# sangminwoo/Temporal-Span-Proposal-Network-VidVRD

Measured on AMD Instinct MI355X. Metric: tracklet-pairs/sec scored (N=32, T=150, D=2048), higher is better.
Workload: dtype f32

## Files before the change

include/tspn_mi355x.h:

```cpp
#ifndef TSPN_MI355X_H
#define TSPN_MI355X_H

#include <stddef.h>
#include <stdint.h>

#ifdef __cplusplus
extern "C" {
#endif

#define TSPN_ABI_VERSION 7

enum {
  TSPN_OK = 0,
  TSPN_EINVAL = -1,
  TSPN_EUNSUPPORTED = -2,
  TSPN_EWORKSPACE = -3,
  TSPN_ELAUNCH = -4,
  TSPN_EDEVICE = -5
};

#define TSPN_STATUS_WORDS 16
enum {
  TSPN_STATUS_FAULT = 0,
  TSPN_STATUS_FAULT_INFO = 1,
// ... 84 lines not shown
size_t tspn_conv3_tc_wino63_workspace_bytes(int64_t B, int64_t T, int64_t Cin);
int tspn_conv3_tc_wino63_f32(const float* x, int64_t B, int64_t T, int64_t Cin, const float* frag,
                             int64_t M, const float* bias, int relu, float* y,
                             void* workspace, size_t workspace_bytes, void* stream);
int tspn_conv3_tc_wino63_set_piece_form(int form);

size_t tspn_pack_conv3_wino63_f16x3_elements(int64_t M, int64_t Cin, int64_t split);
int tspn_pack_conv3_wino63_f16x3(const float* W, int64_t M, int64_t Cin, int64_t split, int16_t* packed, void* stream);
size_t tspn_conv3_tc_wino63_f16x3_workspace_bytes(int64_t B, int64_t T, int64_t Cin, int64_t M);
int tspn_conv3_tc_wino63_f16x3(const float* x, int64_t B, int64_t T, int64_t Cin, const int16_t* packed,
                               int64_t M, const float* bias, int relu, float* y,
                               void* workspace, size_t workspace_bytes, void* stream);
int tspn_conv3_tc_wino63_f16x3_set_tail_split(int on);


int tspn_heads_f32(int mode, const float* a, const float* b, int64_t lda,
                   const int64_t* ia, const int64_t* ib, int64_t idx_stride, const float* bias,
                   const float* Wh, const float* bh, int64_t H,
                   int64_t P, int64_t C, int64_t T, float* out, void* stream);

int tspn_heads_pairgrid_f32(const float* y, int64_t B, int64_t N, int64_t C, int64_t T,
                            const float* Wh, const float* bh, int64_t H, float* out,
                            void* stream);

int tspn_temporal_mean_f32(const float* x, int64_t R, int64_t T, int64_t Cdim,
                           int layout_tc, float* out, void* stream);
int tspn_temporal_sum_f32(const float* x, int64_t R, int64_t T, int64_t Cdim, float* out, void* stream);

int tspn_pair_rows_f32(const float* src, int64_t NT, int64_t D, const int64_t* pairs,
                       int64_t P, float* out, void* stream);

int tspn_transpose_td_f32(const float* x, int64_t R, int64_t T, int64_t D, float* out,
                          void* stream);

size_t tspn_decode_topk_workspace_bytes(int64_t S, int64_t P, int64_t topk_pair);
int tspn_decode_topk_f32(const float* rel_logit, const int64_t* pairs,
                         const float* cls_sub, const float* cls_obj, int64_t ld,
                         int64_t seg_rows, int64_t row_mul, int64_t S, int64_t P, int64_t K,
                         int64_t NO, int64_t topk_pair, int64_t topk_seg,
                         float* out_score, int64_t* out_triplet, int64_t* out_pair_tid,
                         void* workspace, size_t workspace_bytes, void* stream);

int tspn_decode_spans_f32(const float* heads, int64_t P, int64_t A, int64_t T,
                          const float* sizes_host, int64_t top_k, double nms_threshold,
                          int64_t pre_nms, int64_t* out_anchor, int64_t* out_span,
                          float* out_span_f, float* out_score, int64_t* out_count, void* stream);
// ... 216 lines not shown
```

temporal-span-proposal-network-vidvrd_amd/_abi.py:

```python
import ctypes
import os
import re
import threading

HERE = os.path.dirname(os.path.abspath(__file__))
ROOT = os.path.dirname(HERE)
LIB_PATH = os.environ.get("TSPN_LIB_PATH") or os.path.join(HERE, "libtspn_mi355x.so")
HEADER_PATH = os.path.join(ROOT, "include", "tspn_mi355x.h")

ABI_VERSION = 7
TSPN_OK = 0
TSPN_EINVAL = -1
TSPN_EUNSUPPORTED = -2
TSPN_EWORKSPACE = -3
TSPN_ELAUNCH = -4
TSPN_EDEVICE = -5
STATUS_WORDS = 16
STATUS_FAULT, STATUS_FAULT_INFO, STATUS_CONV_ERR, STATUS_CONV_CHECKS = 0, 1, 2, 3
FAULT_HANDOVER = 1
CONV_CHECK_HOT_OFFSET, CONV_CHECK_SCRATCH_BYTES = 256, 256 + 256 * 64
GEOM_CHANNELS = 8
CONV_DIRECT, CONV_WINOGRAD63, CONV_WINOGRAD63_F16X3 = 0, 1, 2

_c_f32p = ctypes.c_void_p
# ... 45 lines not shown
    "tspn_status_selftest": (_int, [_vp, _vp]),
    "tspn_conv3_spot_check_f32": (_int, [_vp, _i64, _i64, _i64, _vp, _i64, _i64, _i64, _vp, _int, _vp, _i64, _vp, _i64, _vp]),
    "tspn_predicate_head_workspace_bytes": (_sz, [_i64, _i64, _i64]),
    "tspn_predicate_head_f32": (_int, [_vp, _i64, _i64, _i64, _vp, _vp, _i64, _vp, _int, _vp, _sz, _vp]),
    "tspn_predicate_head_norm_workspace_bytes": (_sz, [_i64, _i64, _i64, _i64, _i64, _i64]),
    "tspn_predicate_head_norm_f32": (_int, [_vp, _i64, _i64, _i64, _vp, _vp, _i64, _i64, _i64, _i64, _vp, _int,
                                            _vp, _sz, _vp]),
    "tspn_feature_preprocess_f32": (_int, [_vp, _i64, _i64, _i64, _i64, _i64, _i64, _vp]),
    "tspn_proposal_pair_filter_i64": (_int, [_vp, _vp, _vp, _vp, _i64, _vp, _vp, _vp, _vp]),
    "tspn_gather_rows_f32": (_int, [_vp, _i64, _i64, _vp, _i64, _i64, _vp, _vp]),
    "tspn_ppn_pair_matrix_topk_f32": (_int, [_vp, _i64, _i64, _i64, _i64, _i64,
                                             _vp, _vp, _vp, _vp, _vp, _vp, _vp, _vp,
                                             _i64, _vp, _vp, _vp]),
    "tspn_traj_iou_f32": (_int, [_vp, _i64, _vp, _i64, _i64, _i64, _vp, _vp]),
    "tspn_traj_iou_tail_f64": (_int, [_vp, _vp, _vp, _i64, _i64, _i64, _vp, _vp]),
    "tspn_pair_index_i64": (_int, [_i64, _i64, _vp, _vp]),
    "tspn_pair_gather_f32": (_int, [_vp, _vp, _i64, _i64, _i64, _vp, _i64, _vp, _vp, _vp]),
    "tspn_pack_conv3_f32": (_int, [_vp, _i64, _i64, _i64, _vp, _vp]),
    "tspn_conv3_f32": (_int, [_vp, _i64, _i64, _i64, _vp, _i64, _vp, _int, _vp, _vp]),
    "tspn_conv3_tc_f32": (_int, [_vp, _i64, _i64, _i64, _vp, _i64, _vp, _int, _vp, _vp]),
    "tspn_heads_f32": (_int, [_int, _vp, _vp, _i64, _vp, _vp, _i64, _vp, _vp, _vp, _i64, _i64, _i64,
                              _i64, _vp, _vp]),
    "tspn_heads_pairgrid_f32": (_int, [_vp, _i64, _i64, _i64, _i64, _vp, _vp, _i64, _vp, _vp]),
    "tspn_temporal_mean_f32": (_int, [_vp, _i64, _i64, _i64, _int, _vp, _vp]),
    "tspn_temporal_sum_f32": (_int, [_vp, _i64, _i64, _i64, _vp, _vp]),
    "tspn_pair_rows_f32": (_int, [_vp, _i64, _i64, _vp, _i64, _vp, _vp]),
    "tspn_transpose_td_f32": (_int, [_vp, _i64, _i64, _i64, _vp, _vp]),
    "tspn_decode_topk_workspace_bytes": (_sz, [_i64, _i64, _i64]),
    "tspn_decode_topk_f32": (_int, [_vp, _vp, _vp, _vp, _i64, _i64, _i64, _i64, _i64, _i64, _i64, _i64, _i64,
                                    _vp, _vp, _vp, _vp, _sz, _vp]),
    "tspn_decode_spans_f32": (_int, [_vp, _i64, _i64, _i64, ctypes.POINTER(ctypes.c_float), _i64,
                                     ctypes.c_double, _i64, _vp, _vp, _vp, _vp, _vp, _vp]),
    "tspn_forward_fused_workspace_bytes": (_sz, [ctypes.POINTER(FusedDesc)]),
    "tspn_forward_fused_f32": (_int, [ctypes.POINTER(FusedDesc), _vp]),
    "tspn_temporal_encoder_heads_f32": (_int, [_vp, _i64, _i64, _i64, _vp, _vp, _vp, _vp, _i64,
                                               _vp, _vp, _vp]),
    "tspn_pack_conv2d_f32": (_int, [_vp, _i64, _i64, _i64, _i64, _vp, _vp]),
    "tspn_conv2d_nhwc_f32": (_int, [_vp, _i64, _i64, _i64, _i64, _vp, _i64, _i64, _i64, _i64, _i64, _vp, _vp,
                                    _int, _vp, _vp]),
    "tspn_pack_conv2d_frag_f32": (_int, [_vp, _i64, _i64, _i64, _i64, _vp, _vp]),
    "tspn_conv2d_nhwc_frag_f32": (_int, [_vp, _i64, _i64, _i64, _i64, _vp, _i64, _i64, _i64, _i64, _i64, _vp, _vp,
                                         _int, _vp, _vp]),
    "tspn_pack_conv2d_frag_bf16": (_int, [_vp, _i64, _i64, _i64, _i64, _vp, _vp]),
    "tspn_conv2d_nhwc_bf16": (_int, [_vp, _i64, _i64, _i64, _i64, _vp, _i64, _i64, _i64, _i64, _i64, _vp, _vp,
                                     _int, _vp, _vp]),
    "tspn_roi_align_nhwc_f32": (_int, [_vp, _i64, _i64, _i64, _i64, _vp, _i64, _i64, ctypes.c_float, _int, _int,
# ... 123 lines not shown
```

temporal-span-proposal-network-vidvrd_amd/build.py:

```python
import glob
import json
import os
import re
import shutil
import subprocess
import sys

HERE = os.path.dirname(os.path.abspath(__file__))
ROOT = os.path.dirname(HERE)
CSRC = os.path.join(HERE, "csrc")
CSRC_EVAL = os.path.join(CSRC, "eval")
CSRC_REL = os.path.join(CSRC, "relations")
CSRC_PAIRLIST = os.path.join(CSRC, "pairlist")
CSRC_SPANBF16 = os.path.join(CSRC, "spanbf16")
CSRC_SPANLOSS = os.path.join(CSRC, "spanloss")
LIB_NAME = "libtspn_mi355x.so"
LIB_PATH = os.path.join(HERE, LIB_NAME)
ARCH = "gfx950"

FLAGS = [
    f"--offload-arch={ARCH}", "-O3", "-std=c++17", "-fPIC",
    "-ffp-contract=off",
    "-fno-gpu-rdc", "-Wall", "-Wno-unused-function",
    "-Rpass-analysis=kernel-resource-usage",
    f"-I{os.path.join(ROOT, 'include')}", f"-I{CSRC}",
]
OBJ_DIR = os.path.join(HERE, "build", "obj")
RES_PATH = os.path.join(HERE, "kernel_resources.json")

NO_SPILL_KERNELS = ("conv3_wino63_kernel", "heads_pairgrid4_kernel", "heads_pairgrid3_kernel",
                    "conv2d_nhwc_frag_kernel", "conv2d_nhwc_bf16_kernel", "conv2d_nhwc_cin4_kernel",
                    "bottleneck_bf16_kernel", "bottleneck_pipe_bf16_kernel", "conv3_bf16_big_kernel", "heads_pairgrid_bf16_kernel",
                    "heads_pairlist_bf16_kernel",
                    "tail_io_bf16_kernel", "bottleneck_block_bf16_kernel")


def sources():
    return sorted(glob.glob(os.path.join(CSRC, "*.hip")) + glob.glob(os.path.join(CSRC_EVAL, "*.hip")) +
                  glob.glob(os.path.join(CSRC_REL, "*.hip")) + glob.glob(os.path.join(CSRC_PAIRLIST, "*.hip")) +
                  glob.glob(os.path.join(CSRC_SPANBF16, "*.hip")) + glob.glob(os.path.join(CSRC_SPANLOSS, "*.hip")))


def _headers():
    return glob.glob(os.path.join(CSRC, "*.h")) + glob.glob(os.path.join(CSRC_EVAL, "*.h")) + \
        glob.glob(os.path.join(CSRC_REL, "*.h")) + glob.glob(os.path.join(CSRC_PAIRLIST, "*.h")) + \
        glob.glob(os.path.join(CSRC_SPANBF16, "*.h")) + glob.glob(os.path.join(CSRC_SPANLOSS, "*.h")) + \
        glob.glob(os.path.join(ROOT, "include", "*.h")) + \
        [os.path.abspath(__file__)]


def needs_build():
    if not os.path.exists(LIB_PATH) or not os.path.exists(RES_PATH):
        return True
    t = os.path.getmtime(LIB_PATH)
    return any(os.path.getmtime(d) > t for d in sources() + _headers())


def _obj_of(src):
    return os.path.join(OBJ_DIR, os.path.basename(src)[:-4] + ".o")


_REMARK = re.compile(r"remark:\s+(Function Name|TotalSGPRs|VGPRs|AGPRs|ScratchSize \[bytes/lane\]|Occupancy \[waves/SIMD\]|"
                     r"SGPRs Spill|VGPRs Spill|LDS Size \[bytes/block\]): (\S+)")
_KEYS = {"TotalSGPRs": "sgprs", "VGPRs": "vgprs", "AGPRs": "agprs", "ScratchSize [bytes/lane]": "scratch_bytes",
         "Occupancy [waves/SIMD]": "occupancy", "SGPRs Spill": "sgpr_spill", "VGPRs Spill": "vgpr_spill",
         "LDS Size [bytes/block]": "lds_bytes"}


def _demangle(names):
# ... 104 lines not shown
```

temporal-span-proposal-network-vidvrd_amd/csrc/tspn_common.h:

```cpp
#pragma once
#include <hip/hip_runtime.h>

#include <atomic>
#include <cstdarg>
#include <cstdint>
#include <cstdio>
#include <initializer_list>

#include "tspn_mi355x.h"

namespace tspn {

char* err_buf();
constexpr int kErrBufLen = 512;

inline int fail(int code, const char* fmt, ...) {
  va_list ap;
  va_start(ap, fmt);
  vsnprintf(err_buf(), kErrBufLen, fmt, ap);
  va_end(ap);
  return code;
}

int status_check(const char* what);
// ... 54 lines not shown
  }
};

int conv3_tc_direct(const float* x, int64_t B, int64_t T, int64_t Cin, const float* packed, int64_t M,
                    const float* bias, int relu, float* y, int64_t ldy, void* stream);
bool wino63_supported(int64_t Cin, int64_t M);
size_t wino63_workspace_bytes(int64_t B, int64_t T, int64_t Cin);
int wino63_input_transform(const float* x, int64_t B, int64_t T, int64_t Cin, void* workspace,
                           size_t workspace_bytes, void* stream, uint64_t* hot = nullptr);
int wino63_contract(const void* workspace, int64_t B, int64_t T, int64_t Cin, const float* frag, int64_t M,
                    const float* bias, int relu, float* y, int64_t ldy, void* stream);
int conv3_tc_wino63(const float* x, int64_t B, int64_t T, int64_t Cin, const float* frag, int64_t M,
                    const float* bias, int relu, float* y, int64_t ldy, void* workspace,
                    size_t workspace_bytes, void* stream);
bool wino63_f16x3_supported(int64_t Cin, int64_t M);
size_t wino63_f16x3_workspace_bytes(int64_t B, int64_t T, int64_t Cin, int64_t M);
int wino63_f16x3_input_transform(const float* x, int64_t B, int64_t T, int64_t Cin, int64_t M, void* workspace,
                                 size_t workspace_bytes, void* stream, uint64_t* hot = nullptr);
int wino63_f16x3_contract(void* workspace, size_t workspace_bytes, int64_t B, int64_t T, int64_t Cin,
                          const int16_t* packed, int64_t M, const float* bias, int relu, float* y, int64_t ldy,
                          void* stream);
int heads_pairgrid(const float* y, int64_t ldt, int64_t B, int64_t N, int64_t C, int64_t T,
                   const float* Wh, const float* bh, int64_t H, float* out, void* stream, float* Wp12 = nullptr);
inline size_t align_up(size_t a, size_t b) { return (a + b - 1) / b * b; }
int linear(const float* x, int64_t P, int64_t F, int64_t ldx, const float* W, int64_t ldw,
           const float* b, int64_t K, float* out, int apply_sigmoid, void* workspace,
           size_t workspace_bytes, void* stream);
size_t pair_predicate_workspace_bytes(int64_t NT, int64_t D, int64_t K);
int pair_predicate(const float* fbar, int64_t NT, int64_t D, const int64_t* pairs, int64_t P,
                   const float* cls_w, const float* cls_b, int64_t K, float* out, void* workspace,
                   size_t workspace_bytes, void* stream);
size_t span_prefix_workspace_bytes(int64_t NT, int64_t T, int64_t D, int64_t K);
int span_prefix_stage(const float* feats, int64_t NT, int64_t T, int64_t D, const float* cls_w, int64_t K,
                      void* workspace, size_t workspace_bytes, void* stream, const float** G_out,
                      const double** PS_out, const char* who);
inline size_t span_cand_bytes(int64_t S, int64_t P, int64_t J, int64_t R) {
  return align_up((size_t)S * P * J * R * sizeof(float), 256);
}
int segment_span_topk(const unsigned* key, const float* sc, const int* ix, const int64_t* pairs, const int64_t* spans,
                      const int64_t* span_counts, const float* cls_logits, int64_t S, int64_t N, int64_t NO, int64_t P,
                      int64_t J, int64_t R, int64_t topk_per_seg, float* out_score, int64_t* out_triplet,
                      int64_t* out_pair_tid, int64_t* out_span, int64_t* out_span_rank, int64_t* out_valid, void* stream,
                      const char* what);

}

// ... 29 lines not shown
```

temporal-span-proposal-network-vidvrd_amd/csrc/tspn_device.h:

```cpp
#pragma once
#include <hip/hip_runtime.h>

namespace tspn_dev {

typedef float f32x2 __attribute__((ext_vector_type(2)));
typedef float f32x4 __attribute__((ext_vector_type(4)));
typedef float f32x16 __attribute__((ext_vector_type(16)));
typedef __bf16 bf16x2 __attribute__((ext_vector_type(2)));
typedef __bf16 bf16x4 __attribute__((ext_vector_type(4)));
typedef __bf16 bf16x8 __attribute__((ext_vector_type(8)));
typedef _Float16 f16x8 __attribute__((ext_vector_type(8)));
typedef short s16x2 __attribute__((ext_vector_type(2)));
typedef unsigned u32x4 __attribute__((ext_vector_type(4)));

template <int AUX = 0>
__device__ __forceinline__ void glds16(const void* g, void* l) {
  __builtin_amdgcn_global_load_lds((const __attribute__((address_space(1))) void*)g,
                                   (__attribute__((address_space(3))) void*)l, 16, 0, AUX);
}
__device__ __forceinline__ void glds4(const void* g, void* l) {
  __builtin_amdgcn_global_load_lds((const __attribute__((address_space(1))) void*)g,
                                   (__attribute__((address_space(3))) void*)l, 4, 0, 0);
}

// ... 21 lines not shown
template <int VM>
__device__ __forceinline__ void wait_w(f32x4& r0, f32x4& r1) {
  asm volatile("s_waitcnt vmcnt(%2)" : "+v"(r0), "+v"(r1) : "n"(VM));
}
template <int N>
__device__ __forceinline__ void wait_vmcnt() {
  asm volatile("s_waitcnt vmcnt(%0)" ::"n"(N) : "memory");
}

__device__ __forceinline__ int xcd_remap(int id, int n) {
  const int q8 = n >> 3, r8 = n & 7, xcd = id & 7;
  return (xcd < r8 ? xcd * (q8 + 1) : r8 * (q8 + 1) + (xcd - r8) * q8) + (id >> 3);
}
__device__ __forceinline__ void grouped_tile(int wg, int GM, int tiles_m, int tiles_n, int& tile_m, int& tile_n) {
  const int group_sz = GM * tiles_n;
  const int group = wg / group_sz;
  const int first_m = group * GM;
  const int gm = min(GM, tiles_m - first_m);
  const int in_group = wg - group * group_sz;
  tile_m = first_m + in_group % gm;
  tile_n = in_group / gm;
}

}
```

temporal-span-proposal-network-vidvrd_amd/csrc/tspn_fused.hip:

```cpp
#include <algorithm>

#include "tspn_common.h"

namespace {

struct FusedLayout {
  size_t xt, y, bias2, fbar, pooled, lin, vt, hwp, hot, total;
  size_t vt_bytes;
  size_t lin_bytes;
};

FusedLayout layout_of(const tspn_fused_desc* d) {
  FusedLayout L{};
  const size_t NT = (size_t)d->B * d->N, T = d->T, D = d->D, C = 2 * D;
  size_t off = 0;
  auto take = [&](size_t bytes) {
    const size_t o = off;
    off += tspn::align_up(bytes, 256);
    return o;
  };
  L.xt = take(NT * D * T * sizeof(float));
  L.y = take(NT * 2 * C * tspn::align_up(T, 4) * sizeof(float));
  L.bias2 = take(2 * C * sizeof(float));
  L.fbar = take(NT * D * sizeof(float));
  L.pooled = take(256);
  L.lin_bytes = tspn::pair_predicate_workspace_bytes((int64_t)NT, (int64_t)D, d->K);
  L.lin = take(L.lin_bytes);
  L.vt_bytes = (D % 32 == 0) ? tspn::wino63_workspace_bytes((int64_t)NT, (int64_t)T, (int64_t)D) : 0;
  if (d->conv_algo == TSPN_CONV_WINOGRAD63_F16X3)
    L.vt_bytes = tspn::wino63_f16x3_workspace_bytes((int64_t)NT, (int64_t)T, (int64_t)D, (int64_t)(2 * C));
  L.vt = take(L.vt_bytes);
  L.hwp = take(C * 12 * sizeof(float));
  L.hot = take(TSPN_CONV_CHECK_SCRATCH_BYTES);
  L.total = off;
  return L;
}

int check_desc(const tspn_fused_desc* d) {
  TSPN_REQUIRE(d != nullptr, TSPN_EINVAL, "tspn_forward_fused: null descriptor");
  TSPN_REQUIRE(d->B >= 0 && d->N >= 0 && d->T > 0 && d->D > 0 && d->A > 0 && d->K > 0 &&
                   d->P >= 0,
               TSPN_EINVAL, "tspn_forward_fused: bad sizes B=%lld N=%lld T=%lld D=%lld A=%lld K=%lld P=%lld",
               (long long)d->B, (long long)d->N, (long long)d->T, (long long)d->D, (long long)d->A,
               (long long)d->K, (long long)d->P);
  TSPN_REQUIRE(3 * d->A <= 16, TSPN_EUNSUPPORTED, "tspn_forward_fused: 3*A=%lld > 16",
               (long long)(3 * d->A));
  return TSPN_OK;
}

}

extern "C" size_t tspn_forward_fused_workspace_bytes(const tspn_fused_desc* d) {
  if (check_desc(d) != TSPN_OK) return 0;
  return layout_of(d).total;
}
// ... 59 lines not shown
  if (f16x3) {
    if ((rc = tspn::wino63_f16x3_input_transform(d->feats, NT, T, D, 2 * C, ws + L.vt, L.vt_bytes, stream, hot_slots)))
      return rc;
  } else if (w63 && (rc = tspn::wino63_input_transform(d->feats, NT, T, D, ws + L.vt, L.vt_bytes, stream, hot_slots))) {
    return rc;
  }
  if (d->ev_conv_begin) (void)hipEventRecord(static_cast<hipEvent_t>(d->ev_conv_begin), s);
  if (f16x3)
    rc = tspn::wino63_f16x3_contract(ws + L.vt, L.vt_bytes, NT, T, D, reinterpret_cast<const int16_t*>(d->conv_packed), 2 * C,
                                     bias2, 0, y, ldy, stream);
  else if (w63)
    rc = tspn::wino63_contract(ws + L.vt, NT, T, D, d->conv_packed, 2 * C, bias2, 0, y, ldy, stream);
  else
    rc = tc ? tspn::conv3_tc_direct(d->feats, NT, T, D, d->conv_packed, 2 * C, bias2, 0, y, ldy, stream)
            : tspn_conv3_f32(xt, NT, D, T, d->conv_packed, 2 * C, bias2, 0, y, stream);
  if (rc) return rc;
  if (d->ev_conv_end) (void)hipEventRecord(static_cast<hipEvent_t>(d->ev_conv_end), s);
  if (guard && (rc = tspn_conv3_spot_check_f32(d->feats, NT, T, D, d->conv_weight, C, C, D, bias2, 0, y, ldy, hot,
                                               d->conv_check, stream)))
    return rc;
  if (d->canonical_pairs) {
    TSPN_REQUIRE(d->P == d->B * d->N * (d->N - 1), TSPN_EINVAL,
                 "tspn_forward_fused: canonical_pairs needs P == B*N*(N-1) (P=%lld)", (long long)d->P);
    if ((rc = tspn::heads_pairgrid(y, ldy, d->B, d->N, C, T, d->head_w, d->head_b, H, d->out_heads,
                                   stream, reinterpret_cast<float*>(ws + L.hwp))))
      return rc;
  } else if ((rc = tspn_heads_f32(1, y, y + C * T, 2 * C, d->pairs, d->pairs + 1, 2, nullptr,
                                  d->head_w, d->head_b, H, d->P, C, T, d->out_heads, stream))) {
    return rc;
  }
  return TSPN_OK;
}

extern "C" int tspn_temporal_encoder_heads_f32(const float* x, int64_t P, int64_t C, int64_t T,
                                               const float* conv_packed, const float* conv_bias,
                                               const float* head_w, const float* head_b, int64_t H,
                                               float* h_ws, float* out_heads, void* stream) {
  if (P == 0) return TSPN_OK;
  TSPN_REQUIRE(x && conv_packed && head_w && h_ws && out_heads, TSPN_EINVAL,
               "tspn_temporal_encoder_heads_f32: null pointer");
  int rc = tspn_conv3_f32(x, P, C, T, conv_packed, C, conv_bias, 1, h_ws, stream);
  if (rc) return rc;
  return tspn_heads_f32(0, h_ws, nullptr, C, nullptr, nullptr, 1, nullptr, head_w, head_b, H, P, C,
                        T, out_heads, stream);
}
```

temporal-span-proposal-network-vidvrd_amd/csrc/tspn_heads.hip:

```cpp
#include <cstdlib>
#include <type_traits>

#include "tspn_common.h"
#include "tspn_device.h"

namespace {

using namespace tspn_dev;

constexpr int NP = 4;
constexpr int WAVES = 4;
constexpr int TB = 32;

template <int MODE, bool VEC2>
__global__ __launch_bounds__(WAVES * 64) void heads_kernel(
    const float* __restrict__ a, const float* __restrict__ b, int64_t lda,
    const int64_t* __restrict__ ia, const int64_t* __restrict__ ib, int64_t istride,
    const float* __restrict__ bias, const float* __restrict__ Wh, const float* __restrict__ bh,
    int H, int64_t P, int C, int T, float* __restrict__ out) {
  const int lane = threadIdx.x & 63;
  const int wave = threadIdx.x >> 6;
  const int n_tblk = (T + TB - 1) / TB;
  const int64_t wave_global = (int64_t)blockIdx.x * WAVES + wave;
  const int64_t group = wave_global / n_tblk;
// ... 84 lines not shown
    if (p >= P) break;
#pragma unroll
    for (int e = 0; e < 4; ++e) {
      const int o = kq * 4 + e;
      if (o >= H) continue;
      const float bo = bh ? bh[o] : 0.f;
      float* dst = out + (p * H + o) * (int64_t)T;
      const float v0 = acc[q][0][e] + bo;
      const float v1 = acc[q][1][e] + bo;
      if (VEC2) {
        if (tA < T) *reinterpret_cast<float2*>(dst + tA) = make_float2(v0, v1);
      } else {
        if (tA < T) dst[tA] = v0;
        if (tB < T) dst[tB] = v1;
      }
    }
  }
}

constexpr int PG_S = 8, PG_O = 8, PG_CK = 16, PG_T = 32;
constexpr int PG_ROWS = PG_S + PG_O;
constexpr int PG_STAGE = PG_ROWS * PG_CK * PG_T;

__device__ __forceinline__ int64_t pair_stage_group(int id, int nsb, int nob, int& sb, int& ob) {
  const int per_group = nsb * nob;
  const int xcd = id & 7, k = id >> 3;
  const int member = k % per_group;
  sb = member / nob;
  ob = member - sb * nob;
  return (int64_t)(k / per_group) * 8 + xcd;
}

template <bool VEC2>
__global__ __launch_bounds__(256, 2) void heads_pairgrid_kernel(
    const float* __restrict__ y, int C, int T, int N, const float* __restrict__ Wh,
    const float* __restrict__ bh, int H, float* __restrict__ out, int ntb, int nob, int nsb,
    int64_t ngroups) {
  extern __shared__ __attribute__((aligned(16))) char smem_raw[];
  float* S = reinterpret_cast<float*>(smem_raw);

  const int tid = threadIdx.x;
  const int lane = tid & 63, wave = tid >> 6;
  const int j = lane & 15, kq = lane >> 4;
  int sb, ob;
  const int64_t G = pair_stage_group(blockIdx.x, nsb, nob, sb, ob);
  if (G >= ngroups) return;
  const int64_t b = G / ntb;
  const int tb = (int)(G - b * ntb);
  const int t0 = tb * PG_T;
  const int64_t rowlen = 2 * (int64_t)C * T;

  const int st_ch = tid >> 4, st_t2 = tid & 15;
  int lt = t0 + 2 * st_t2;
  if (VEC2) lt = min(lt, T - 2); else lt = min(lt, T - 1);
// ... 559 lines not shown
```

temporal-span-proposal-network-vidvrd_amd/ops.py:

```python
import ctypes
import threading

import torch

from . import _abi

__all__ = [
    "predicate_head", "feature_preprocess_", "ppn_pair_matrix_topk", "traj_iou", "traj_iou_tail", "pair_index",
    "pair_gather", "pack_conv3", "conv3", "conv3_tc", "pack_conv3_wino63", "conv3_tc_wino63", "pack_conv3_wino63_f16x3", "conv3_tc_wino63_f16x3", "heads", "heads_pairgrid", "temporal_mean", "temporal_sum", "pair_rows", "transpose_td",
    "forward_fused", "temporal_encoder_heads", "fused_workspace_bytes", "fused_bf16_workspace_bytes", "decode_topk", "decode_spans", "decode_span_relations",
    "span_anchor_labels", "span_loss",
    "cast_bf16", "pack_conv3_bf16", "pack_heads_bf16", "conv3_tc_bf16", "heads_pairgrid_bf16",
    "pair_plan", "heads_pairlist_bf16",
    "transpose_cast_bf16", "temporal_encoder_heads_bf16",
    "temporal_mean_bf16", "forward_fused_bf16", "span_predicate",
    "pack_span_cls_bf16", "span_predicate_bf16", "decode_span_relations_bf16", "bottleneck_block_bf16", "bottleneck_block_proj_bf16", "bottleneck_block_res_bf16",
    "proposal_pair_filter", "gather_rows", "wino63_set_piece_form", "wino63_f16x3_set_tail_split", "conv3_spot_check",
    "pack_conv2d", "pack_conv2d_frag", "conv2d_nhwc", "roi_align_nhwc", "pack_conv2d_frag_bf16", "conv2d_nhwc_bf16", "max_pool_nhwc", "pack_conv2d_frag_cin4", "conv2d_nhwc_cin4", "max_pool_nhwc_bf16", "pack_stem_bf16", "stem_conv_bf16", "stem_pool_bf16", "bottleneck_tail_bf16",
    "eval_traj_volume", "eval_viou", "eval_greedy_match",
    "status_words", "status_fault", "status_clear", "status_selftest",
]


_status_blocks = {}
_status_lock = threading.Lock()


def _status_block(index=None):
    idx = torch.cuda.current_device() if index is None else int(index)
    blk = _status_blocks.get(idx)
    if blk is not None:
        return blk
# ... 437 lines not shown
        if t is not None:
            _dev(t, nm, torch.int64)
    if b is not None:
        _dev(b, "b")
        if b.shape[1:] != a.shape[1:]:
            raise ValueError("heads: a / b shape mismatch")
    if num_pairs is None:
        num_pairs = ia.shape[0] if ia is not None else a.shape[0]
    out = torch.empty((num_pairs, H, T), dtype=torch.float32, device=a.device)
    _abi.check(_abi.lib().tspn_heads_f32(mode, _p(a), _p(b), lda, _p(ia), _p(ib), 1, _p(bias),
                                         _p(head_w), _p(head_b), H, num_pairs, C, T, _p(out), _stream()))
    return out


def heads_pairgrid(y, B, N, head_w, head_b):
    _dev(y, "y"); _dev(head_w, "head_w")
    NT, C2, T = y.shape
    C, H = C2 // 2, head_w.shape[0]
    if NT != B * N or head_w.shape[1] != C:
        raise ValueError("heads_pairgrid: shape mismatch")
    out = torch.empty((B * N * max(N - 1, 0), H, T), dtype=torch.float32, device=y.device)
    _abi.check(_abi.lib().tspn_heads_pairgrid_f32(_p(y), B, N, C, T, _p(head_w), _p(head_b), H, _p(out),
                                                  _stream()))
    return out


def temporal_mean(x, layout_tc):
    _dev(x, "x")
    if layout_tc:
        R, T, Cd = x.shape
    else:
        R, Cd, T = x.shape
    out = torch.empty((R, Cd), dtype=torch.float32, device=x.device)
    _abi.check(_abi.lib().tspn_temporal_mean_f32(_p(x), R, T, Cd, 1 if layout_tc else 0, _p(out), _stream()))
    return out


def temporal_sum(x):
    _dev(x, "x")
    R, T, Cd = x.shape
    out = torch.empty((R, Cd), dtype=torch.float32, device=x.device)
    _abi.check(_abi.lib().tspn_temporal_sum_f32(_p(x), R, T, Cd, _p(out), _stream()))
    return out


def pair_rows(src, pairs):
# ... 1014 lines not shown
```

Baseline: 1.190 million.

## Add f16x3 split-precision MFMA kernel for pairgrid heads in fused forward

Adds a new pair-head kernel that splits the relu(u+v) activations and the per-row scaled head weights into fp16 hi/lo parts and accumulates three MFMA products, emulating f32 accuracy on fp16 matrix cores instead of running the f32 pairgrid kernel. Weights are pre-packed into MFMA fragments with per-head power-of-two scales. The kernel falls back to an exact scalar path when values are non-finite or out of range. The fused forward selects it when the Winograd f16x3 conv path is active and H==12. This trades extra packing work and an approximation with range checks for much higher matrix throughput.

```diff
diff --git a/include/tspn_mi355x.h b/include/tspn_mi355x.h
--- a/include/tspn_mi355x.h
+++ b/include/tspn_mi355x.h
@@ -130,6 +130,12 @@
 int tspn_heads_pairgrid_f32(const float* y, int64_t B, int64_t N, int64_t C, int64_t T,
                             const float* Wh, const float* bh, int64_t H, float* out,
                             void* stream);
+
+size_t tspn_heads_pairgrid_f16x3_split_bytes(int64_t C, int64_t H);
+int tspn_heads_pairgrid_f16x3_set_force_exact(int on);
+int tspn_heads_pairgrid_f16x3(const float* y, int64_t ldt, int64_t B, int64_t N, int64_t C, int64_t T,
+                              const float* Wh, const float* bh, int64_t H, void* split_buf, size_t split_bytes,
+                              float* out, void* stream);
 
 int tspn_temporal_mean_f32(const float* x, int64_t R, int64_t T, int64_t Cdim,
                            int layout_tc, float* out, void* stream);
diff --git a/temporal-span-proposal-network-vidvrd_amd/_abi.py b/temporal-span-proposal-network-vidvrd_amd/_abi.py
--- a/temporal-span-proposal-network-vidvrd_amd/_abi.py
+++ b/temporal-span-proposal-network-vidvrd_amd/_abi.py
@@ -91,6 +91,9 @@
     "tspn_heads_f32": (_int, [_int, _vp, _vp, _i64, _vp, _vp, _i64, _vp, _vp, _vp, _i64, _i64, _i64,
                               _i64, _vp, _vp]),
     "tspn_heads_pairgrid_f32": (_int, [_vp, _i64, _i64, _i64, _i64, _vp, _vp, _i64, _vp, _vp]),
+    "tspn_heads_pairgrid_f16x3_split_bytes": (_sz, [_i64, _i64]),
+    "tspn_heads_pairgrid_f16x3_set_force_exact": (_int, [_int]),
+    "tspn_heads_pairgrid_f16x3": (_int, [_vp, _i64, _i64, _i64, _i64, _i64, _vp, _vp, _i64, _vp, _sz, _vp, _vp]),
     "tspn_temporal_mean_f32": (_int, [_vp, _i64, _i64, _i64, _int, _vp, _vp]),
     "tspn_temporal_sum_f32": (_int, [_vp, _i64, _i64, _i64, _vp, _vp]),
     "tspn_pair_rows_f32": (_int, [_vp, _i64, _i64, _vp, _i64, _vp, _vp]),
diff --git a/temporal-span-proposal-network-vidvrd_amd/build.py b/temporal-span-proposal-network-vidvrd_amd/build.py
--- a/temporal-span-proposal-network-vidvrd_amd/build.py
+++ b/temporal-span-proposal-network-vidvrd_amd/build.py
@@ -13,6 +13,7 @@
 CSRC_REL = os.path.join(CSRC, "relations")
 CSRC_PAIRLIST = os.path.join(CSRC, "pairlist")
 CSRC_SPANBF16 = os.path.join(CSRC, "spanbf16")
+CSRC_PAIRF16 = os.path.join(CSRC, "pairf16")
 CSRC_SPANLOSS = os.path.join(CSRC, "spanloss")
 LIB_NAME = "libtspn_mi355x.so"
 LIB_PATH = os.path.join(HERE, LIB_NAME)
@@ -31,20 +32,22 @@
 NO_SPILL_KERNELS = ("conv3_wino63_kernel", "heads_pairgrid4_kernel", "heads_pairgrid3_kernel",
                     "conv2d_nhwc_frag_kernel", "conv2d_nhwc_bf16_kernel", "conv2d_nhwc_cin4_kernel",
                     "bottleneck_bf16_kernel", "bottleneck_pipe_bf16_kernel", "conv3_bf16_big_kernel", "heads_pairgrid_bf16_kernel",
-                    "heads_pairlist_bf16_kernel",
+                    "heads_pairlist_bf16_kernel", "heads_pair_f16x3_kernel",
                     "tail_io_bf16_kernel", "bottleneck_block_bf16_kernel")
 
 
 def sources():
     return sorted(glob.glob(os.path.join(CSRC, "*.hip")) + glob.glob(os.path.join(CSRC_EVAL, "*.hip")) +
                   glob.glob(os.path.join(CSRC_REL, "*.hip")) + glob.glob(os.path.join(CSRC_PAIRLIST, "*.hip")) +
-                  glob.glob(os.path.join(CSRC_SPANBF16, "*.hip")) + glob.glob(os.path.join(CSRC_SPANLOSS, "*.hip")))
+                  glob.glob(os.path.join(CSRC_SPANBF16, "*.hip")) + glob.glob(os.path.join(CSRC_SPANLOSS, "*.hip")) +
+                  glob.glob(os.path.join(CSRC_PAIRF16, "*.hip")))
 
 
 def _headers():
     return glob.glob(os.path.join(CSRC, "*.h")) + glob.glob(os.path.join(CSRC_EVAL, "*.h")) + \
         glob.glob(os.path.join(CSRC_REL, "*.h")) + glob.glob(os.path.join(CSRC_PAIRLIST, "*.h")) + \
         glob.glob(os.path.join(CSRC_SPANBF16, "*.h")) + glob.glob(os.path.join(CSRC_SPANLOSS, "*.h")) + \
+        glob.glob(os.path.join(CSRC_PAIRF16, "*.h")) + \
         glob.glob(os.path.join(ROOT, "include", "*.h")) + \
         [os.path.abspath(__file__)]
 
diff --git a/temporal-span-proposal-network-vidvrd_amd/csrc/pairf16/tspn_heads_pair_f16x3.hip b/temporal-span-proposal-network-vidvrd_amd/csrc/pairf16/tspn_heads_pair_f16x3.hip
--- /dev/null
+++ b/temporal-span-proposal-network-vidvrd_amd/csrc/pairf16/tspn_heads_pair_f16x3.hip
@@ -0,0 +1,340 @@
+#include "tspn_common.h"
+#include "tspn_device.h"
+
+namespace {
+using namespace tspn_dev;
+
+constexpr int PF_S = 8, PF_O = 8, PF_T = 32, PF_CK = 32;
+constexpr int PF_ROWS = PF_S + PF_O;
+constexpr int PF_STAGE = PF_ROWS * PF_CK * PF_T;
+constexpr int PF_THREADS = 64 * PF_S;
+constexpr size_t PF_SMEM = sizeof(float) * 2 * PF_STAGE;
+constexpr int PF_HDR_BYTES = 256;
+constexpr int PF_KSTEP_BYTES = 2 * 64 * 16;
+constexpr float PF_LO = 2048.f, PF_LO_INV = 1.f / 2048.f;
+constexpr float PF_RANGE = 16384.f;
+
+typedef _Float16 f16x2 __attribute__((ext_vector_type(2)));
+
+std::atomic<int> g_force_exact{0};
+
+__device__ __forceinline__ unsigned split_lo(unsigned h2, float as0, float as1) {
+  unsigned d;
+  const float neg = -PF_LO;
+  asm("v_fma_mixlo_f16 %0, %1, %2, %3 op_sel_hi:[1,0,0]" : "=v"(d) : "v"(h2), "s"(neg), "v"(as0));
+  asm("v_fma_mixhi_f16 %0, %1, %2, %3 op_sel:[1,0,0] op_sel_hi:[1,0,0]" : "+v"(d) : "v"(h2), "s"(neg), "v"(as1));
+  return d;
+}
+
+__global__ __launch_bounds__(1024) void pairf16_scale_kernel(const float* __restrict__ Wh, int C, int H,
+                                                            unsigned* __restrict__ hdr) {
+  __shared__ unsigned bad_s[16];
+  const int lane = threadIdx.x & 63, h = threadIdx.x >> 6;
+  float mx = 0.f;
+  bool finite = true;
+  if (h < H) {
+    for (int c = lane; c < C; c += 64) {
+      const float a = fabsf(Wh[(int64_t)h * C + c]);
+      finite = finite && (a < __builtin_inff());
+      mx = fmaxf(mx, a);
+    }
+  }
+#pragma unroll
+  for (int o = 32; o > 0; o >>= 1) mx = fmaxf(mx, __shfl_xor(mx, o, 64));
+  const bool all_finite = __all(finite);
+  int e = 0;
+  (void)frexpf(mx, &e);
+  const bool bad = h < H && (!all_finite || !(mx >= 0x1p-100f) || e > 100);
+  if (lane == 0) {
+    bad_s[h] = bad ? 1u : 0u;
+    hdr[1 + h] = __float_as_uint((h < H && !bad) ? ldexpf(1.f, e) : 1.f);
+  }
+  __syncthreads();
+  if (threadIdx.x == 0) {
+    unsigned f = 0;
+    for (int i = 0; i < 16; ++i) f |= bad_s[i];
+    hdr[0] = f;
+  }
+  if (threadIdx.x >= 17 && threadIdx.x < PF_HDR_BYTES / 4) hdr[threadIdx.x] = 0;
+}
+
+__global__ __launch_bounds__(64) void pairf16_pack_kernel(const float* __restrict__ Wh, int C, int H,
+                                                         const unsigned* __restrict__ hdr, u32x4* __restrict__ frag) {
+  const int lane = threadIdx.x, h = lane & 15, kg = lane >> 4;
+  const float scale = 1.f / __uint_as_float(hdr[1 + h]);
+  unsigned hi[4], lo[4];
+#pragma unroll
+  for (int ip = 0; ip < 4; ++ip) {
+    f16x2 wh, wl;
+#pragma unroll
+    for (int e = 0; e < 2; ++e) {
+      const int c = blockIdx.x * PF_CK + kg + 4 * (2 * ip + e);
+      const float w = (h < H) ? Wh[(int64_t)h * C + c] * scale : 0.f;
+      const _Float16 a = (_Float16)w;
+      wh[e] = a;
+      wl[e] = (_Float16)((w - (float)a) * PF_LO);
+    }
+    hi[ip] = __builtin_bit_cast(unsigned, wh);
+    lo[ip] = __builtin_bit_cast(unsigned, wl);
+  }
+  frag[(int64_t)blockIdx.x * 128 + lane] = u32x4{hi[0], hi[1], hi[2], hi[3]};
+  frag[(int64_t)blockIdx.x * 128 + 64 + lane] = u32x4{lo[0], lo[1], lo[2], lo[3]};
+}
+
+__device__ __noinline__ void exact_tile(const float* __restrict__ y, int64_t ldt, int C, int T, int N, int H,
+                                        const float* __restrict__ Wh, const float* __restrict__ bh,
+                                        float* __restrict__ out, int64_t b, int sb, int ob, int t0) {
+  const int t = t0 + (threadIdx.x & 31);
+  if (t >= T) return;
+  for (int idx = threadIdx.x >> 5; idx < PF_S * PF_O * H; idx += PF_THREADS / 32) {
+    const int pair = idx / H, h = idx - pair * H;
+    const int s = sb * PF_S + (pair >> 3), o = ob * PF_O + (pair & 7);
+    if (s >= N || o >= N || s == o) continue;
+    const float* up = y + ((b * N + s) * 2 * (int64_t)C) * ldt + t;
+    const float* vp = y + ((b * N + o) * 2 * (int64_t)C + C) * ldt + t;
+    const float* w = Wh + (int64_t)h * C;
+    float sum = 0.f;
+    for (int c = 0; c < C; ++c) sum = __builtin_fmaf(w[c], tspn::relu_f32(up[c * ldt] + vp[c * ldt]), sum);
+    const int64_t p = b * N * (int64_t)(N - 1) + (int64_t)s * (N - 1) + o - (o > s ? 1 : 0);
+    out[(p * H + h) * (int64_t)T + t] = sum + (bh ? bh[h] : 0.f);
+  }
+}
+
+__global__ __launch_bounds__(PF_THREADS, 1) void heads_pair_f16x3_kernel(
+    const float* __restrict__ y, int64_t ldt, int C, int T, int N, int H, const float* __restrict__ Wh,
+    const float* __restrict__ bh, const unsigned* __restrict__ hdr, const u32x4* __restrict__ frag,
+    float* __restrict__ out, int ntb, int nob, int nsb, int64_t ngroups, int force_exact) {
+  extern __shared__ __attribute__((aligned(16))) char smem_raw[];
+  float* S = reinterpret_cast<float*>(smem_raw);
+
+  const int tid = threadIdx.x;
+  const int lane = tid & 63;
+  const int wave = __builtin_amdgcn_readfirstlane(tid >> 6);
+  const int j = lane & 15, kg = lane >> 4;
+  int sb, ob;
+  const int64_t G = pair_stage_group(blockIdx.x, nsb, nob, sb, ob);
+  if (G >= ngroups) return;
+  const int64_t b = G / ntb;
+  const int t0 = (int)(G - b * ntb) * PF_T;
+  const int64_t rowlen = 2 * (int64_t)C * ldt;
+
+  if (force_exact | (int)hdr[0]) {
+    exact_tile(y, ldt, C, T, N, H, Wh, bh, out, b, sb, ob, t0);
+    return;
+  }
+
+  const __amdgpu_buffer_rsrc_t rsrc_y = buffer_rsrc(y + b * N * rowlen, (int)(unsigned)((int64_t)N * rowlen * 4));
+  unsigned voff[2];
+  const unsigned loff = (unsigned)((lane >> 3) * ldt + min((int64_t)t0 + (lane & 7) * 4, ldt - 4));
+#pragma unroll
+  for (int r = 0; r < 2; ++r) {
+    const int row = 2 * wave + r;
+    const int local = row < PF_S ? sb * PF_S + row : ob * PF_O + (row - PF_S);
+    const int64_t trk = min(local, N - 1);
+    voff[r] = (unsigned)((trk * rowlen + (row < PF_S ? 0 : (int64_t)C * ldt) + loff) * 4);
+  }
+  const int piece_bytes = (int)(8 * ldt * 4);
+  int y_soff = 0;
+  auto stage = [&](int buf) {
+#pragma unroll
+    for (int r = 0; r < 2; ++r) {
+#pragma unroll
+      for (int q = 0; q < 4; ++q)
+        bglds16(rsrc_y, voff[r], y_soff + q * piece_bytes, S + buf * PF_STAGE + ((2 * wave + r) * PF_CK + 8 * q) * PF_T);
+    }
+    y_soff += 4 * piece_bytes;
+  };
+
+  f32x4 acc_hi[PF_O][2], acc_lo[PF_O][2];
+#pragma unroll
+  for (int o = 0; o < PF_O; ++o) {
+#pragma unroll
+    for (int cb = 0; cb < 2; ++cb) acc_hi[o][cb] = acc_lo[o][cb] = f32x4{0.f, 0.f, 0.f, 0.f};
+  }
+
+  const int nk = C / PF_CK;
+  stage(0);
+  u32x4 wh = frag[lane], wl = frag[64 + lane];
+  asm volatile("s_waitcnt vmcnt(0)" ::: "memory");
+  __syncthreads();
+  const float* urow = S + (wave * PF_CK + kg) * PF_T + 2 * j;
+  const float* vrow = S + (PF_S * PF_CK + kg) * PF_T + 2 * j;
+  const float* trow = vrow + wave * PF_CK * PF_T;
+  float mu = 0.f, mv = 0.f;
+  for (int k = 0; k < nk; ++k) {
+    const int buf = k & 1;
+    u32x4 whn = wh, wln = wl;
+    if (k + 1 < nk) {
+      stage(buf ^ 1);
+      whn = frag[(int64_t)(k + 1) * 128 + lane];
+      wln = frag[(int64_t)(k + 1) * 128 + 64 + lane];
+    }
+    const float* ub = urow + buf * PF_STAGE;
+    const float* vb = vrow + buf * PF_STAGE;
+    const float* tb = trow + buf * PF_STAGE;
+    f32x2 u[8];
+#pragma unroll
+    for (int i = 0; i < 8; ++i) {
+      u[i] = *reinterpret_cast<const f32x2*>(ub + 4 * i * PF_T);
+      const f32x2 vt = *reinterpret_cast<const f32x2*>(tb + 4 * i * PF_T);
+      mu = __builtin_elementwise_maximum(__builtin_elementwise_maximum(mu, __builtin_fabsf(u[i][0])), __builtin_fabsf(u[i][1]));
+      mv = __builtin_elementwise_maximum(__builtin_elementwise_maximum(mv, __builtin_fabsf(vt[0])), __builtin_fabsf(vt[1]));
+    }
+    const f16x8 a_hi = __builtin_bit_cast(f16x8, wh), a_lo = __builtin_bit_cast(f16x8, wl);
+    f32x2 v[8], vn[8];
+    u32x4 fh[2], fl[2], gh[2], gl[2];
+#pragma unroll
+    for (int i = 0; i < 8; ++i) v[i] = *reinterpret_cast<const f32x2*>(vb + 4 * i * PF_T);
+#pragma unroll
+    for (int o = 0; o <= PF_O; ++o) {
+      if (o + 1 < PF_O) {
+#pragma unroll
+        for (int i = 0; i < 8; ++i) vn[i] = *reinterpret_cast<const f32x2*>(vb + ((o + 1) * PF_CK + 4 * i) * PF_T);
+      }
+      if (o < PF_O) {
+        f32x2 a[8], as[8];
+#pragma unroll
+        for (int i = 0; i < 8; ++i) {
+          const f32x2 x = u[i] + v[i];
+          a[i] = f32x2{tspn::relu_f32(x[0]), tspn::relu_f32(x[1])};
+          as[i] = a[i] * PF_LO;
+        }
+#pragma unroll
+        for (int cb = 0; cb < 2; ++cb) {
+          unsigned ph[4], pl[4];
+#pragma unroll
+          for (int ip = 0; ip < 4; ++ip) {
+            const f16x2 h = __builtin_convertvector(f32x2{a[2 * ip][cb], a[2 * ip + 1][cb]}, f16x2);
+            ph[ip] = __builtin_bit_cast(unsigned, h);
+            pl[ip] = split_lo(ph[ip], as[2 * ip][cb], as[2 * ip + 1][cb]);
+          }
+          gh[cb] = u32x4{ph[0], ph[1], ph[2], ph[3]};
+          gl[cb] = u32x4{pl[0], pl[1], pl[2], pl[3]};
+        }
+      }
+      if (o > 0) {
+        const f16x8 h0 = __builtin_bit_cast(f16x8, fh[0]), h1 = __builtin_bit_cast(f16x8, fh[1]);
+        const f16x8 l0 = __builtin_bit_cast(f16x8, fl[0]), l1 = __builtin_bit_cast(f16x8, fl[1]);
+        acc_hi[o - 1][0] = __builtin_amdgcn_mfma_f32_16x16x32_f16(a_hi, h0, acc_hi[o - 1][0], 0, 0, 0);
+        acc_lo[o - 1][0] = __builtin_amdgcn_mfma_f32_16x16x32_f16(a_hi, l0, acc_lo[o - 1][0], 0, 0, 0);
+        acc_hi[o - 1][1] = __builtin_amdgcn_mfma_f32_16x16x32_f16(a_hi, h1, acc_hi[o - 1][1], 0, 0, 0);
+        acc_lo[o - 1][1] = __builtin_amdgcn_mfma_f32_16x16x32_f16(a_hi, l1, acc_lo[o - 1][1], 0, 0, 0);
+        acc_lo[o - 1][0] = __builtin_amdgcn_mfma_f32_16x16x32_f16(a_lo, h0, acc_lo[o - 1][0], 0, 0, 0);
+        acc_lo[o - 1][1] = __builtin_amdgcn_mfma_f32_16x16x32_f16(a_lo, h1, acc_lo[o - 1][1], 0, 0, 0);
+      }
+      if (o > 0 && o < PF_O) {
+#define TSPN_G                                         \
+  __builtin_amdgcn_sched_group_barrier(0x008, 1, 0);   \
+  __builtin_amdgcn_sched_group_barrier(0x100, 2, 0);   \
+  __builtin_amdgcn_sched_group_barrier(0x002, 10, 0);
+        TSPN_G TSPN_G TSPN_G TSPN_G TSPN_G TSPN_G
+#undef TSPN_G
+      }
+      __builtin_amdgcn_sched_barrier(0);
+#pragma unroll
+      for (int cb = 0; cb < 2; ++cb) {
+        fh[cb] = gh[cb];
+        fl[cb] = gl[cb];
+      }
+#pragma unroll
+      for (int i = 0; i < 8; ++i) v[i] = vn[i];
+    }
+    wh = whn;
+    wl = wln;
+    asm volatile("s_waitcnt vmcnt(0)" ::: "memory");
+    __syncthreads();
+  }
+
+  const int tA = t0 + 2 * j;
+  const int s = sb * PF_S + wave;
+  const bool bad = tA < T && ((s < N && !(mu <= PF_RANGE)) || (ob * PF_O + wave < N && !(mv <= PF_RANGE)));
+  if (__syncthreads_or(bad)) {
+    exact_tile(y, ldt, C, T, N, H, Wh, bh, out, b, sb, ob, t0);
+    return;
+  }
+
+  if (tA >= T || s >= N) return;
+  float inv[4], bias[4];
+#pragma unroll
+  for (int r = 0; r < 4; ++r) {
+    const int h = 4 * kg + r;
+    inv[r] = __uint_as_float(hdr[1 + h]);
+    bias[r] = (h < H && bh) ? bh[h] : 0.f;
+  }
+#pragma unroll
+  for (int o = 0; o < PF_O; ++o) {
+    const int ot = ob * PF_O + o;
+    if (ot >= N || ot == s) continue;
+    const int64_t p = b * N * (int64_t)(N - 1) + (int64_t)s * (N - 1) + ot - (ot > s ? 1 : 0);
+#pragma unroll
+    for (int r = 0; r < 4; ++r) {
+      const int h = 4 * kg + r;
+      if (h >= H) continue;
+      const float v0 = __builtin_fmaf(acc_lo[o][0][r], PF_LO_INV, acc_hi[o][0][r]) * inv[r] + bias[r];
+      const float v1 = __builtin_fmaf(acc_lo[o][1][r], PF_LO_INV, acc_hi[o][1][r]) * inv[r] + bias[r];
+      *reinterpret_cast<float2*>(out + (p * H + h) * (int64_t)T + tA) = make_float2(v0, v1);
+    }
+  }
+}
+
+}
+
+size_t tspn::heads_pair_f16x3_split_bytes(int64_t C, int64_t H) {
+  if (C <= 0 || C % PF_CK != 0 || C >= (1 << 24) || H <= 0 || H > 16) return 0;
+  return (size_t)PF_HDR_BYTES + (size_t)(C / PF_CK) * PF_KSTEP_BYTES;
+}
+
+bool tspn::heads_pair_f16x3_supported(const float* y, int64_t ldt, int64_t N, int64_t C, int64_t T, int64_t H,
+                                      const float* out) {
+  return H > 0 && H <= 16 && C > 0 && C % PF_CK == 0 && C < (1 << 24) && T > 0 && T % 2 == 0 && ldt >= T && ldt % 4 == 0 &&
+         ldt < (1 << 24) && N < (1 << 15) && N * 2 * C * ldt * 4 < (1LL << 31) && tspn::aligned16(y) &&
+         (reinterpret_cast<uintptr_t>(out) & 7) == 0;
+}
+
+int tspn::heads_pair_f16x3(const float* y, int64_t ldt, int64_t B, int64_t N, int64_t C, int64_t T, const float* Wh,
+                           const float* bh, int64_t H, void* split_buf, size_t split_bytes, float* out, void* stream) {
+  const char* what = "tspn_heads_pairgrid_f16x3";
+  TSPN_REQUIRE(B >= 0 && N >= 0 && C > 0 && T > 0 && ldt >= T, TSPN_EINVAL,
+               "%s: bad sizes B=%lld N=%lld C=%lld T=%lld ldt=%lld", what, (long long)B, (long long)N, (long long)C,
+               (long long)T, (long long)ldt);
+  TSPN_REQUIRE(H > 0 && H <= 16, TSPN_EUNSUPPORTED, "%s: H=%lld not in [1,16]", what, (long long)H);
+  if (B == 0 || N < 2) return TSPN_OK;
+  TSPN_REQUIRE(y && Wh && out && split_buf, TSPN_EINVAL, "%s: null pointer", what);
+  TSPN_REQUIRE(tspn::heads_pair_f16x3_supported(y, ldt, N, C, T, H, out), TSPN_EUNSUPPORTED,
+               "%s: needs C %% 32 == 0, even T, ldt %% 4 == 0, a video's projections below 2 GB, y 16-byte and out 8-byte "
+               "aligned", what);
+  const size_t need = tspn::heads_pair_f16x3_split_bytes(C, H);
+  TSPN_REQUIRE(split_bytes >= need, TSPN_EWORKSPACE, "%s: split buffer %zu < %zu bytes", what, split_bytes, need);
+  TSPN_REQUIRE(tspn::aligned16(split_buf), TSPN_EINVAL, "%s: split buffer must be 16-byte aligned", what);
+  const int ntb = (int)tspn::ceil_div(T, PF_T);
+  const int nsb = (int)tspn::ceil_div(N, PF_S), nob = (int)tspn::ceil_div(N, PF_O);
+  const int64_t ngroups = B * ntb;
+  const int64_t nwg = tspn::ceil_div(ngroups, 8) * 8 * nsb * nob;
+  TSPN_REQUIRE(nwg < (1LL << 31), TSPN_EUNSUPPORTED, "%s: grid too large", what);
+  hipStream_t s = TSPN_STREAM(stream);
+  unsigned* hdr = static_cast<unsigned*>(split_buf);
+  u32x4* frag = reinterpret_cast<u32x4*>(static_cast<char*>(split_buf) + PF_HDR_BYTES);
+  hipLaunchKernelGGL(pairf16_scale_kernel, dim3(1), dim3(1024), 0, s, Wh, (int)C, (int)H, hdr);
+  hipLaunchKernelGGL(pairf16_pack_kernel, dim3((unsigned)(C / PF_CK)), dim3(64), 0, s, Wh, (int)C, (int)H, hdr, frag);
+  static tspn::LdsLimit lds;
+  if (int rc = lds.ensure(reinterpret_cast<const void*>(heads_pair_f16x3_kernel), PF_SMEM, what)) return rc;
+  hipLaunchKernelGGL(heads_pair_f16x3_kernel, dim3((unsigned)nwg), dim3(PF_THREADS), PF_SMEM, s, y, ldt, (int)C, (int)T,
+                     (int)N, (int)H, Wh, bh, hdr, frag, out, ntb, nob, nsb, ngroups,
+                     g_force_exact.load(std::memory_order_relaxed));
+  return tspn::check_launch(what);
+}
+
+extern "C" size_t tspn_heads_pairgrid_f16x3_split_bytes(int64_t C, int64_t H) {
+  return tspn::heads_pair_f16x3_split_bytes(C, H);
+}
+
+extern "C" int tspn_heads_pairgrid_f16x3_set_force_exact(int on) {
+  TSPN_REQUIRE(on == 0 || on == 1, TSPN_EINVAL, "tspn_heads_pairgrid_f16x3_set_force_exact: on must be 0 or 1");
+  return g_force_exact.exchange(on, std::memory_order_relaxed);
+}
+
+extern "C" int tspn_heads_pairgrid_f16x3(const float* y, int64_t ldt, int64_t B, int64_t N, int64_t C, int64_t T,
+                                         const float* Wh, const float* bh, int64_t H, void* split_buf, size_t split_bytes,
+                                         float* out, void* stream) {
+  return tspn::heads_pair_f16x3(y, ldt, B, N, C, T, Wh, bh, H, split_buf, split_bytes, out, stream);
+}
diff --git a/temporal-span-proposal-network-vidvrd_amd/csrc/tspn_common.h b/temporal-span-proposal-network-vidvrd_amd/csrc/tspn_common.h
--- a/temporal-span-proposal-network-vidvrd_amd/csrc/tspn_common.h
+++ b/temporal-span-proposal-network-vidvrd_amd/csrc/tspn_common.h
@@ -100,6 +100,10 @@
                           void* stream);
 int heads_pairgrid(const float* y, int64_t ldt, int64_t B, int64_t N, int64_t C, int64_t T,
                    const float* Wh, const float* bh, int64_t H, float* out, void* stream, float* Wp12 = nullptr);
+size_t heads_pair_f16x3_split_bytes(int64_t C, int64_t H);
+bool heads_pair_f16x3_supported(const float* y, int64_t ldt, int64_t N, int64_t C, int64_t T, int64_t H, const float* out);
+int heads_pair_f16x3(const float* y, int64_t ldt, int64_t B, int64_t N, int64_t C, int64_t T, const float* Wh,
+                     const float* bh, int64_t H, void* split_buf, size_t split_bytes, float* out, void* stream);
 inline size_t align_up(size_t a, size_t b) { return (a + b - 1) / b * b; }
 int linear(const float* x, int64_t P, int64_t F, int64_t ldx, const float* W, int64_t ldw,
            const float* b, int64_t K, float* out, int apply_sigmoid, void* workspace,
diff --git a/temporal-span-proposal-network-vidvrd_amd/csrc/tspn_device.h b/temporal-span-proposal-network-vidvrd_amd/csrc/tspn_device.h
--- a/temporal-span-proposal-network-vidvrd_amd/csrc/tspn_device.h
+++ b/temporal-span-proposal-network-vidvrd_amd/csrc/tspn_device.h
@@ -67,4 +67,13 @@
   tile_n = in_group / gm;
 }
 
+__device__ __forceinline__ int64_t pair_stage_group(int id, int nsb, int nob, int& sb, int& ob) {
+  const int per_group = nsb * nob;
+  const int xcd = id & 7, k = id >> 3;
+  const int member = k % per_group;
+  sb = member / nob;
+  ob = member - sb * nob;
+  return (int64_t)(k / per_group) * 8 + xcd;
 }
+
+}
diff --git a/temporal-span-proposal-network-vidvrd_amd/csrc/tspn_fused.hip b/temporal-span-proposal-network-vidvrd_amd/csrc/tspn_fused.hip
--- a/temporal-span-proposal-network-vidvrd_amd/csrc/tspn_fused.hip
+++ b/temporal-span-proposal-network-vidvrd_amd/csrc/tspn_fused.hip
@@ -5,8 +5,9 @@
 namespace {
 
 struct FusedLayout {
-  size_t xt, y, bias2, fbar, pooled, lin, vt, hwp, hot, total;
+  size_t xt, y, bias2, fbar, pooled, lin, vt, hwp, hot, psplit, total;
   size_t vt_bytes;
+  size_t psplit_bytes;
   size_t lin_bytes;
 };
 
@@ -31,6 +32,9 @@
     L.vt_bytes = tspn::wino63_f16x3_workspace_bytes((int64_t)NT, (int64_t)T, (int64_t)D, (int64_t)(2 * C));
   L.vt = take(L.vt_bytes);
   L.hwp = take(C * 12 * sizeof(float));
+  L.psplit_bytes = (d->conv_algo == TSPN_CONV_WINOGRAD63_F16X3 && 3 * d->A == 12)
+                       ? tspn::heads_pair_f16x3_split_bytes((int64_t)C, 12) : 0;
+  L.psplit = take(L.psplit_bytes);
   L.hot = take(TSPN_CONV_CHECK_SCRATCH_BYTES);
   L.total = off;
   return L;
@@ -136,9 +140,14 @@
   if (d->canonical_pairs) {
     TSPN_REQUIRE(d->P == d->B * d->N * (d->N - 1), TSPN_EINVAL,
                  "tspn_forward_fused: canonical_pairs needs P == B*N*(N-1) (P=%lld)", (long long)d->P);
-    if ((rc = tspn::heads_pairgrid(y, ldy, d->B, d->N, C, T, d->head_w, d->head_b, H, d->out_heads,
-                                   stream, reinterpret_cast<float*>(ws + L.hwp))))
-      return rc;
+    if (f16x3 && H == 12 && L.psplit_bytes > 0 &&
+        tspn::heads_pair_f16x3_supported(y, ldy, d->N, C, T, H, d->out_heads))
+      rc = tspn::heads_pair_f16x3(y, ldy, d->B, d->N, C, T, d->head_w, d->head_b, H, ws + L.psplit, L.psplit_bytes,
+                                  d->out_heads, stream);
+    else
+      rc = tspn::heads_pairgrid(y, ldy, d->B, d->N, C, T, d->head_w, d->head_b, H, d->out_heads, stream,
+                                reinterpret_cast<float*>(ws + L.hwp));
+    if (rc) return rc;
   } else if ((rc = tspn_heads_f32(1, y, y + C * T, 2 * C, d->pairs, d->pairs + 1, 2, nullptr,
                                   d->head_w, d->head_b, H, d->P, C, T, d->out_heads, stream))) {
     return rc;
diff --git a/temporal-span-proposal-network-vidvrd_amd/csrc/tspn_heads.hip b/temporal-span-proposal-network-vidvrd_amd/csrc/tspn_heads.hip
--- a/temporal-span-proposal-network-vidvrd_amd/csrc/tspn_heads.hip
+++ b/temporal-span-proposal-network-vidvrd_amd/csrc/tspn_heads.hip
@@ -130,14 +130,6 @@
 constexpr int PG_ROWS = PG_S + PG_O;
 constexpr int PG_STAGE = PG_ROWS * PG_CK * PG_T;
 
-__device__ __forceinline__ int64_t pair_stage_group(int id, int nsb, int nob, int& sb, int& ob) {
-  const int per_group = nsb * nob;
-  const int xcd = id & 7, k = id >> 3;
-  const int member = k % per_group;
-  sb = member / nob;
-  ob = member - sb * nob;
-  return (int64_t)(k / per_group) * 8 + xcd;
-}
 
 template <bool VEC2>
 __global__ __launch_bounds__(256, 2) void heads_pairgrid_kernel(
diff --git a/temporal-span-proposal-network-vidvrd_amd/ops.py b/temporal-span-proposal-network-vidvrd_amd/ops.py
--- a/temporal-span-proposal-network-vidvrd_amd/ops.py
+++ b/temporal-span-proposal-network-vidvrd_amd/ops.py
@@ -7,7 +7,8 @@
 
 __all__ = [
     "predicate_head", "feature_preprocess_", "ppn_pair_matrix_topk", "traj_iou", "traj_iou_tail", "pair_index",
-    "pair_gather", "pack_conv3", "conv3", "conv3_tc", "pack_conv3_wino63", "conv3_tc_wino63", "pack_conv3_wino63_f16x3", "conv3_tc_wino63_f16x3", "heads", "heads_pairgrid", "temporal_mean", "temporal_sum", "pair_rows", "transpose_td",
+    "pair_gather", "pack_conv3", "conv3", "conv3_tc", "pack_conv3_wino63", "conv3_tc_wino63", "pack_conv3_wino63_f16x3", "conv3_tc_wino63_f16x3", "heads", "heads_pairgrid", "heads_pairgrid_f16x3", "heads_pairgrid_f16x3_split_bytes",
+    "heads_pairgrid_f16x3_set_force_exact", "temporal_mean", "temporal_sum", "pair_rows", "transpose_td",
     "forward_fused", "temporal_encoder_heads", "fused_workspace_bytes", "fused_bf16_workspace_bytes", "decode_topk", "decode_spans", "decode_span_relations",
     "span_anchor_labels", "span_loss",
     "cast_bf16", "pack_conv3_bf16", "pack_heads_bf16", "conv3_tc_bf16", "heads_pairgrid_bf16",
@@ -491,6 +492,33 @@
     out = torch.empty((B * N * max(N - 1, 0), H, T), dtype=torch.float32, device=y.device)
     _abi.check(_abi.lib().tspn_heads_pairgrid_f32(_p(y), B, N, C, T, _p(head_w), _p(head_b), H, _p(out),
                                                   _stream()))
+    return out
+
+
+def heads_pairgrid_f16x3_split_bytes(C, H):
+    return int(_abi.lib().tspn_heads_pairgrid_f16x3_split_bytes(int(C), int(H)))
+
+
+def heads_pairgrid_f16x3_set_force_exact(on):
+    prev = _abi.lib().tspn_heads_pairgrid_f16x3_set_force_exact(int(on))
+    if prev < 0:
+        _abi.check(prev)
+    return prev
+
+
+def heads_pairgrid_f16x3(y, B, N, head_w, head_b, T=None, split_buf=None, out=None):
+    _dev(y, "y"); _dev(head_w, "head_w")
+    NT, C2, ldt = y.shape
+    T = ldt if T is None else int(T)
+    C, H = C2 // 2, head_w.shape[0]
+    if NT != B * N or head_w.shape[1] != C:
+        raise ValueError("heads_pairgrid_f16x3: shape mismatch")
+    if split_buf is None:
+        split_buf = torch.empty(max(heads_pairgrid_f16x3_split_bytes(C, H), 16), dtype=torch.uint8, device=y.device)
+    if out is None:
+        out = torch.empty((B * N * max(N - 1, 0), H, T), dtype=torch.float32, device=y.device)
+    _abi.check(_abi.lib().tspn_heads_pairgrid_f16x3(_p(y), ldt, B, N, C, T, _p(head_w), _p(head_b), H, _p(split_buf),
+                                                    split_buf.numel(), _p(out), _stream()))
     return out
 
 
```

Measured after the change: 1.219 million (median of 6 runs). 1.02x the previous value.
